# wtaylor17/ImageCFGen-Pytorch

Measured on AMD Instinct MI355X. Metric: ALI training images/sec (E+G+D step), MorphoMNIST bs=512/GPU, higher is better.
Workload: dtype f32; 1 GPU; image_scms/mnist.py ALI iteration (EG step + 2 D steps + diagnostics), MorphoMNIST 28x28x1 synthetic, bs=512/GPU, fp32 MFMA, mode=stepper+hipgraph; global_batch=512, parallelism=dp1

## Files before the change

imagecfgen-pytorch_amd/csrc/ali_common.h:

```cpp
#pragma once
#include <hip/hip_runtime.h>
#include <stdint.h>
#include <stdio.h>
#include <stdlib.h>
#include "../../include/ali_hip.h"

namespace ali {

void set_error(const char* fmt, ...);

inline int check_launch(const char* what) {
  hipError_t e = hipGetLastError();
  if (e != hipSuccess) {
    set_error("%s: %s", what, hipGetErrorString(e));
    return ALI_ERR_LAUNCH;
  }
  return ALI_OK;
}

struct Tuning {
  int bm, bn, splitk;
  long long wgrad_small;
  int wgrad_blocks, wgrad_scap;
  int no_first_wgrad;
  int no_order;
  int tile_m_scale;
  int wbm, wbn;
  int no_xcd;
  int no_s2_first;
  int no_dma16;
  int no_t1_mfma;
};
inline Tuning read_tuning() {
  {
    auto num = [](const char* name) -> long long { const char* e = getenv(name); return e ? atoll(e) : 0; };
    Tuning v;
    v.bm = (int)num("ALI_BM"); v.bn = (int)num("ALI_BN"); v.splitk = (int)num("ALI_SPLITK");
    v.wgrad_small = getenv("ALI_WGRAD_SMALL") ? num("ALI_WGRAD_SMALL") : -1;
    v.wgrad_blocks = (int)num("ALI_WGRAD_BLOCKS"); v.wgrad_scap = (int)num("ALI_WGRAD_SCAP");
    v.no_order = (int)num("ALI_NO_ORDER");
    v.no_first_wgrad = (int)num("ALI_NO_FIRST_WGRAD");
    v.tile_m_scale = (int)num("ALI_TILE_M_SCALE");
    v.wbm = (int)num("ALI_WBM"); v.wbn = (int)num("ALI_WBN");
    v.no_t1_mfma = (int)num("ALI_NO_T1_MFMA");
    v.no_xcd = (int)num("ALI_NO_XCD");
    v.no_s2_first = (int)num("ALI_NO_S2_FIRST");
    v.no_dma16 = (int)num("ALI_NO_DMA16");
    return v;
  }
}
inline Tuning& tuning_slot() {
  static Tuning t = read_tuning();
  return t;
}
inline const Tuning& tuning() { return tuning_slot(); }

using f32x4 = __attribute__((ext_vector_type(4))) float;
using f32x16 = __attribute__((ext_vector_type(16))) float;

constexpr int kMaxTaps = 28;
constexpr int kNumCU = 256;

constexpr size_t kWsReserved = ALI_WS_RESERVED;
inline void* ws_payload(void* ws) { return ws ? static_cast<char*>(ws) + kWsReserved : nullptr; }
inline size_t ws_payload_bytes(size_t bytes) { return bytes > kWsReserved ? bytes - kWsReserved : 0; }

#define ST(s) ((hipStream_t)(s))
inline bool aligned16(const void* p) { return (reinterpret_cast<uintptr_t>(p) & 15) == 0; }

constexpr uint64_t kCounterMul = 0xD1B54A32D192ED03ull;
__host__ __device__ __forceinline__ uint64_t mix64(uint64_t z) {
  z += 0x9E3779B97F4A7C15ull;
  z = (z ^ (z >> 30)) * 0xBF58476D1CE4E5B9ull;
  z = (z ^ (z >> 27)) * 0x94D049BB133111EBull;
  return z ^ (z >> 31);
}

constexpr uint64_t kLatentStream = 0x4C4154454E545A31ull;
__device__ __forceinline__ void normal_pair(uint64_t key, uint64_t pair, float& c, float& s) {
  const uint64_t r = mix64(key ^ pair);
// ... 27 lines not shown
```

imagecfgen-pytorch_amd/csrc/gconv.hip:

```cpp
#include "ali_common.h"
#include <algorithm>
#include <vector>
#include <stdarg.h>
#include <stdlib.h>
#include <string.h>
#include <type_traits>

namespace ali {

static thread_local char g_err[512] = "";
void set_error(const char* fmt, ...) {
  va_list ap;
  va_start(ap, fmt);
  vsnprintf(g_err, sizeof(g_err), fmt, ap);
  va_end(ap);
}
const char* get_error() { return g_err; }

constexpr int BK = 32;
constexpr int LDK = BK + 4;
constexpr int kMaxGrid = 5;

struct Phase {
  int Hq, Wq;
  int oh0, ow0, ostep;
  int mult;
  int nr, ns, M, tile0, pixmajor;
  signed char dh[kMaxGrid], dw[kMaxGrid];
  unsigned char wr[kMaxGrid], ws[kMaxGrid];
};

struct GDesc {
  const float* in;
  const float* w;
  float* out;
  float* ws;
  int* ctr;
  AliEpilogue ep;
  int B, Hin, Win, Cin;
  int Hout, Wout, Cout, ldo;
  int ldw, S;
  int nphase, splitk, kt_per_split;
  int ntile_m, ntile_n;
  int lin1d;
  int xcd_chunk;
  int tail_u0, tail_split;
  const int* order;
  int ldi;
  int f16;
  const _Float16* in16;
  const _Float16* w16;
  _Float16* out16;
  unsigned in_bytes, w_bytes;
  long long out_elems;
  Phase ph[4];
};

__device__ __attribute__((aligned(64))) float g_zero[16];

__device__ __forceinline__ void fast_divmod(int m, int dv, float rcp, int& q, int& r) {
  q = (int)((float)m * rcp);
  r = m - q * dv;
  if (r < 0) { --q; r += dv; }
  else if (r >= dv) { ++q; r -= dv; }
}

using f16x4 = __attribute__((ext_vector_type(4))) _Float16;
using f16x8 = __attribute__((ext_vector_type(8))) _Float16;
constexpr int LDH = 40;

template <int BM, int BN, int WAVES_M, int WAVES_N, int MODE, int F16 = 0, int NT = 256>
__device__ __forceinline__ void gconv_body(const GDesc& d, const int bx_, const int by_, const int bz_, const int u_) {
  constexpr int WM = BM / WAVES_M, WN = BN / WAVES_N;
  constexpr int TM = WM / 32, TN = WN / 32;
  constexpr int RPP = NT / 8;
  constexpr int AP = BM / RPP, BP = BN / RPP;
  constexpr bool DMA = F16 == 3;
  constexpr int LDX = DMA ? 32 : LDK;
  constexpr int NL = AP + BP;
  constexpr int NMF = 16 * TM * TN;
  static_assert(WAVES_M * WAVES_N * 64 == NT, "one wave per 64 threads");

  __shared__ __attribute__((aligned(1024))) float As[2][BM * LDX];
  __shared__ __attribute__((aligned(1024))) float Bs[2][BN * LDX];
  __shared__ int s_rowoff[BM];
  __shared__ int s_rowimg[BM];
  __shared__ int s_tap[kMaxTaps];
  __shared__ __attribute__((aligned(16))) int s_live[kMaxTaps + 8][4];
  __shared__ unsigned s_tapmask;

  const int t = threadIdx.x;
  const int lane = t & 63, wave = t >> 6;
  const int wm = wave / WAVES_N, wn = wave % WAVES_N;

  int bx = bx_, by = by_, bz = bz_, nsplit = d.splitk;
  if (d.lin1d) {
    int u = u_;
    bz = 0;
    nsplit = 1;
    if (u >= d.tail_u0) {
      const int r = u - d.tail_u0;
      u = d.tail_u0 + r / d.tail_split;
      bz = r - (r / d.tail_split) * d.tail_split;
      nsplit = d.tail_split;
    }
    if (d.xcd_chunk) {
      const int id = (u & 7) * d.xcd_chunk + (u >> 3);
      if (id >= d.ntile_m * d.ntile_n) return;
      bx = id / d.ntile_n;
      by = id - bx * d.ntile_n;
    } else if (d.order) {
      const int full = (d.ntile_m >> 3) << 3;
      int rank;
      if (u < full * d.ntile_n) {
        const int grp = u / (8 * d.ntile_n), rem = u - grp * 8 * d.ntile_n;
        rank = grp * 8 + (rem & 7);
        by = rem >> 3;
      } else {
        const int r = u - full * d.ntile_n;
        rank = full + r / d.ntile_n;
        by = r - (r / d.ntile_n) * d.ntile_n;
      }
      bx = d.order[rank];
    } else {
      by = u / d.ntile_m;
      bx = u - by * d.ntile_m;
    }
  }
  int p = 0;
#pragma unroll
  for (int i = 1; i < 4; ++i)
    if (i < d.nphase && bx >= d.ph[i].tile0) p = i;
  const Phase& P = d.ph[p];
  const int m0 = (bx - P.tile0) * BM;
  const int n0 = by * BN;
  const int Cin = d.Cin, Hin = d.Hin, Win = d.Win;
  const int ntaps = P.nr * P.ns;

  if (t < kMaxTaps) {
    int v = 0;
    if (t < ntaps) {
      const int ir = t / P.ns, is = t - ir * P.ns;
      v = (P.dh[ir] & 0xff) | ((P.dw[is] & 0xff) << 8) | (((int)P.wr[ir] * d.S + (int)P.ws[is]) << 16);
    }
    s_tap[t] = v;
  }
  if (t == 0) s_tapmask = 0u;

  const float rW = 1.0f / (float)P.Wq, rH = 1.0f / (float)P.Hq, rB = 1.0f / (float)d.B;
  auto decode = [&](int m, int& img, int& qh, int& qw) {
    if (P.pixmajor) {
      int pix;
      fast_divmod(m, d.B, rB, pix, img);
      fast_divmod(pix, P.Wq, rW, qh, qw);
    } else {
      int t2;
      fast_divmod(m, P.Wq, rW, t2, qw);
      fast_divmod(t2, P.Hq, rH, img, qh);
    }
  };
  for (int r = t; r < BM; r += NT) {
    const int m = m0 + r;
    int off = -1, img = 0;
    if (m < P.M) {
      int qh, qw;
      decode(m, img, qh, qw);
      off = ((img * d.Hout + P.oh0 + qh * P.ostep) * d.Wout + (P.ow0 + qw * P.ostep)) * d.ldo;
    }
    s_rowoff[r] = off;
    s_rowimg[r] = img;
  }

  const int c4 = t & 7;
  const int r0 = t >> 3;
  int aoff[AP], aih[AP], aiw[AP];
  unsigned amask[AP];
  unsigned blockmask = 0u;
#pragma unroll
  for (int i = 0; i < AP; ++i) {
    const int m = m0 + r0 + RPP * i;
    const bool valid = m < P.M;
    int qw, qh, img;
    decode(valid ? m : 0, img, qh, qw);
    aih[i] = qh * P.mult;
    aiw[i] = qw * P.mult;
    aoff[i] = ((img * Hin + aih[i]) * Win + aiw[i]) * d.ldi;
    unsigned wbits = 0u, mk = 0u;
    for (int is = 0; is < P.ns; ++is)
      if ((unsigned)(aiw[i] + P.dw[is]) < (unsigned)Win) wbits |= 1u << is;
    for (int ir = 0; ir < P.nr; ++ir)
      if ((unsigned)(aih[i] + P.dh[ir]) < (unsigned)Hin) mk |= wbits << (ir * P.ns);
    amask[i] = valid ? mk : 0u;
    blockmask |= amask[i];
  }
  __syncthreads();
  if (c4 == 0 && blockmask) atomicOr(&s_tapmask, blockmask);
  __syncthreads();
  const unsigned tapmask = s_tapmask;

  float bias_pre[TN];
#pragma unroll
  for (int j = 0; j < TN; ++j) {
    const int n = n0 + wn * WN + j * 32 + (lane & 31);
    bias_pre[j] = (d.ep.bias && n < d.Cout) ? d.ep.bias[n] : 0.f;
  }

  f32x16 acc[TM][TN];
#pragma unroll
  for (int i = 0; i < TM; ++i)
#pragma unroll
    for (int j = 0; j < TN; ++j)
#pragma unroll
      for (int r = 0; r < 16; ++r) acc[i][j][r] = 0.f;

  f32x4 ra[AP], rb[BP];
  f32x4 ra1[AP], rb1[BP];
  auto store_tile = [&](int buf) {
#pragma unroll
    for (int i = 0; i < AP; ++i) *reinterpret_cast<f32x4*>(&As[buf][(r0 + RPP * i) * LDK + c4 * 4]) = ra[i];
#pragma unroll
    for (int j = 0; j < BP; ++j) *reinterpret_cast<f32x4*>(&Bs[buf][(r0 + RPP * j) * LDK + c4 * 4]) = rb[j];
  };
  const int lrow = lane & 31, lh = lane >> 5;
  const float* Ab = &As[0][(wm * WM + lrow) * LDK + lh * 4];
  const float* Bb = &Bs[0][(wn * WN + lrow) * LDK + lh * 4];
  f32x4 fa[2][TM], fb[2][TN];

  if (MODE >= 2) {
    if (MODE == 3) {
      if (t < kMaxTaps + 8) {
        const bool live = t < ntaps && ((tapmask >> t) & 1u);
        const int tv = s_tap[t < kMaxTaps ? t : 0];
        const int dh = (signed char)(tv & 0xff), dw = (signed char)((tv >> 8) & 0xff), wt = (tv >> 16) & 0xff;
        s_live[t][0] = ((dh * Win + dw) * d.ldi) * 4;
        s_live[t][1] = live ? (wt * Cin) * 4 : (int)0xFFFFFF00u;
        s_live[t][2] = live ? (int)(1u << t) : 0;
        s_live[t][3] = 0;
      }
    } else if (t < ntaps && ((tapmask >> t) & 1u)) {
      const int pos = __popc(tapmask & ((1u << t) - 1u));
      const int tv = s_tap[t];
      const int dh = (signed char)(tv & 0xff), dw = (signed char)((tv >> 8) & 0xff), wt = (tv >> 16) & 0xff;
      s_live[pos][0] = ((dh * Win + dw) * d.ldi) * 4;
      s_live[pos][1] = (wt * Cin) * 4;
      s_live[pos][2] = (int)(1u << t);
      s_live[pos][3] = 0;
    }
    __syncthreads();
    const int tpt = MODE == 3 ? BK / Cin : 1;
    const int tsub = MODE == 3 ? (c4 * 4) / Cin : 0;
    const int ccol = MODE == 3 ? (c4 * 4) % Cin : c4 * 4;
    const int cpt = MODE == 3 ? 1 : Cin / BK;
    const int nlive = MODE == 3 ? (ntaps + tpt - 1) / tpt : __popc(tapmask);
    const int total = nlive * cpt;
    const int per = (total + nsplit - 1) / nsplit;
    const int qb = bz * per;
    const int qe = min(total, qb + per);

    const __amdgpu_buffer_rsrc_t rin = __builtin_amdgcn_make_buffer_rsrc((void*)d.in, 0, d.in_bytes, 0x00020000);
    const __amdgpu_buffer_rsrc_t rw = __builtin_amdgcn_make_buffer_rsrc((void*)d.w, 0, d.w_bytes, 0x00020000);
    constexpr unsigned OOB = 0xFFFFFF00u;
    unsigned aoffB[AP], woffB[BP];
#pragma unroll
    for (int i = 0; i < AP; ++i) aoffB[i] = (unsigned)(aoff[i] + ccol) * 4u;
#pragma unroll
    for (int j = 0; j < BP; ++j) {
      const int n = n0 + r0 + RPP * j;
      woffB[j] = n < d.Cout ? (unsigned)(((long long)n * d.ldw + ccol) * 4) : OOB;
    }
    struct Ctx { int doff, woff; unsigned bit; };
    auto tile_ctx = [&](int li, int ch, bool live) -> Ctx {
      const int lc = MODE == 3 ? (li < nlive ? li * tpt + tsub : 0)
                               : (li < nlive ? li : (nlive > 0 ? nlive - 1 : 0));
      const int4 ti = *reinterpret_cast<const int4*>(&s_live[lc][0]);
      if (MODE == 3 && li >= nlive) live = false;
      Ctx cx;
// ... 231 lines not shown
              for (int j = 0; j < TN; ++j)
                acc[i][j] = __builtin_amdgcn_mfma_f32_32x32x16_f16(ha[i], hb[j], acc[i][j], 0, 0, 0);
          }
          store_tile16(buf ^ 1, OTHER);
          __syncthreads();
          buf ^= 1;
          ++q;
        };
        while (q < qe) {
          iteration16(Set0{}, Set1{});
          if (q >= qe) break;
          iteration16(Set1{}, Set0{});
        }
      }
    } else if (qb < qe) {
      int q = qb;
      int li = q / cpt, ch = q - li * cpt;
      {
        const Ctx c0 = tile_ctx(li, ch, true);
#pragma unroll
        for (int i = 0; i < AP; ++i) load_a(c0, i, Set0{});
#pragma unroll
        for (int j = 0; j < BP; ++j) load_b(c0, j, Set0{});
        if (++ch == cpt) { ch = 0; ++li; }
        const Ctx c1 = tile_ctx(li, ch, q + 1 < qe);
#pragma unroll
        for (int i = 0; i < AP; ++i) load_a(c1, i, Set1{});
#pragma unroll
        for (int j = 0; j < BP; ++j) load_b(c1, j, Set1{});
      }
      store_tile(0);
      if (++ch == cpt) { ch = 0; ++li; }
      Ctx cxn = tile_ctx(li, ch, q + 2 < qe);
      __syncthreads();
      int buf = 0;
      auto iteration = [&](auto FETCH) {
        constexpr int fetch = decltype(FETCH)::value;
        const float* Ac = Ab + buf * (BM * LDK);
        const float* Bc = Bb + buf * (BN * LDK);
        float* Aw = &As[buf ^ 1][r0 * LDK + c4 * 4];
        float* Bw = &Bs[buf ^ 1][r0 * LDK + c4 * 4];
        Ctx cxn2 = cxn;
#pragma unroll
        for (int i = 0; i < TM; ++i) fa[0][i] = *reinterpret_cast<const f32x4*>(Ac + i * 32 * LDK);
#pragma unroll
        for (int j = 0; j < TN; ++j) fb[0][j] = *reinterpret_cast<const f32x4*>(Bc + j * 32 * LDK);
#pragma unroll
        for (int s = 0; s < NMF; ++s) {
          const int kg = s / (4 * TM * TN), e = (s / (TM * TN)) & 3, i = (s / TN) % TM, j = s % TN;
          acc[i][j] = __builtin_amdgcn_mfma_f32_32x32x2f32(fa[kg & 1][i][e], fb[kg & 1][j][e], acc[i][j], 0, 0, 0);
          __builtin_amdgcn_sched_barrier(0);
          {
            constexpr int Q = NMF / 4;
            if (s < Q) {
#pragma unroll
              for (int x = 0; x < NL; ++x) {
                if ((x * Q) / NL != s) continue;
                if (x < AP) load_a(cxn, x, FETCH); else load_b(cxn, x - AP, FETCH);
              }
            }
          }
          {
            const int sg = s - kg * 4 * TM * TN - 1;
            if (kg < 3 && sg >= 0 && sg < TM + TN) {
              if (sg < TM)
                fa[(kg + 1) & 1][sg] = *reinterpret_cast<const f32x4*>(Ac + sg * 32 * LDK + (kg + 1) * 8);
              else
                fb[(kg + 1) & 1][sg - TM] = *reinterpret_cast<const f32x4*>(Bc + (sg - TM) * 32 * LDK + (kg + 1) * 8);
            }
          }
          if (s == NMF / 2) {
            if (++ch == cpt) { ch = 0; ++li; }
            cxn2 = tile_ctx(li, ch, q + 3 < qe);
          }
          {
            constexpr int Q = NMF / 4;
            const int sw = s - 3 * Q;
            if (sw >= 0) {
#pragma unroll
              for (int x = 0; x < NL; ++x) {
                if ((x * Q) / NL != sw) continue;
                if (x < AP) *reinterpret_cast<f32x4*>(Aw + RPP * x * LDK) = fetch ? ra[x] : ra1[x];
                else *reinterpret_cast<f32x4*>(Bw + RPP * (x - AP) * LDK) = fetch ? rb[x - AP] : rb1[x - AP];
              }
            }
          }
          __builtin_amdgcn_sched_barrier(0);
        }
        cxn = cxn2;
        __syncthreads();
        buf ^= 1;
        ++q;
      };
      while (q < qe) {
        iteration(Set0{});
        if (q >= qe) break;
        iteration(Set1{});
      }
    }
  } else {
    const int Ktot = ntaps * Cin;
    const int nkt = (Ktot + BK - 1) / BK;
    const int kt_begin = bz * d.kt_per_split;
    const int kt_end = min(nkt, kt_begin + d.kt_per_split);
    const float* wptr[BP];
    bool bvalid[BP];
#pragma unroll
    for (int j = 0; j < BP; ++j) {
      const int n = n0 + r0 + RPP * j;
      bvalid[j] = n < d.Cout;
      wptr[j] = d.w + (long long)(bvalid[j] ? n : 0) * d.ldw;
    }
    auto tile_live = [&](int kt) -> bool {
      const int tlo = (kt * BK) / Cin;
      int thi = (kt * BK + BK - 1) / Cin;
      if (thi > ntaps - 1) thi = ntaps - 1;
      const unsigned span = (thi - tlo + 1) >= 32 ? 0xffffffffu : ((1u << (thi - tlo + 1)) - 1u);
      return ((tapmask >> tlo) & span) != 0u;
    };
    auto next_live = [&](int kt) -> int {
      while (kt < kt_end && !tile_live(kt)) ++kt;
      return kt;
    };
    auto load_tile = [&](int kt, bool live) {
      const int kflat = kt * BK + c4 * 4;
      if (MODE == 1) {
        const bool kvalid = live && kflat < Ktot;
        const int tap = kvalid ? kflat / Cin : 0;
        const int c = kflat - tap * Cin;
        const int tv = s_tap[tap];
// ... 436 lines not shown
  if (dma) S = 1;
  if (blocks > (long long)(kWsReserved / sizeof(int)) || !ws) S = 1;
  while (S > 1 && (long long)S * d.out_elems * 4 >= 0xFF000000LL) --S;
  d.splitk = S;
  d.kt_per_split = (max_nkt + S - 1) / S;
  if (d.kt_per_split < 1) d.kt_per_split = 1;
  d.ntile_m = tiles;
  d.ntile_n = ntile_n;
  d.tail_split = 1;
  d.tail_u0 = 0;
  if (S == 1 && uni && ws && blocks > kNumCU && blocks < 4 * kNumCU && blocks <= (long long)(kWsReserved / sizeof(int))
      && tuning().splitk == 0 && !dma) {
    const int R = (int)(blocks % kNumCU);
    int Sr = 1;
    while (R > 0 && Sr * 2 <= 8 && Sr * 2 * R <= kNumCU && max_nkt / (Sr * 2) >= 4) Sr *= 2;
    if (Sr > 1 && (size_t)Sr * d.out_elems * sizeof(float) <= ws_payload_bytes(ws_bytes) &&
        (long long)Sr * d.out_elems * 4 < 0xFF000000LL) {
      d.tail_split = Sr;
      d.tail_u0 = (int)(blocks - R);
    }
  }
  d.order = nullptr;
  if (d.ep.tile_order && uni && S == 1 && d.ep.tile_order_n == tiles && tuning().no_order == 0)
    d.order = reinterpret_cast<const int*>(d.ep.tile_order);
  d.lin1d = (d.tail_split > 1 || d.order) ? 1 : 0;
  if (d.tail_split == 1) d.tail_u0 = (int)blocks;
  d.xcd_chunk = 0;
  bool img_major = d.nphase >= 1;
  for (int i = 0; i < d.nphase; ++i) img_major = img_major && !d.ph[i].pixmajor;
  if (!d.lin1d && S == 1 && !job && img_major && blocks >= 8LL * kNumCU && blocks < (1LL << 30) && tuning().no_xcd == 0) {
    d.xcd_chunk = (int)((blocks + 7) / 8);
    d.lin1d = 1;
  }
  d.ctr = reinterpret_cast<int*>(ws);
  d.ws = reinterpret_cast<float*>(ws_payload(ws));
  dim3 grid(tiles, ntile_n, S), block(256);
  if (d.lin1d) grid = dim3(d.tail_u0 + (int)(blocks - d.tail_u0) * d.tail_split, 1, 1);
  if (d.xcd_chunk) grid = dim3(8 * d.xcd_chunk, 1, 1);
  if (tiles == 0 || d.out_elems == 0) return ALI_OK;
  const bool f16 = d.f16 && uni;
  const bool op16 = f16 && d.in16 && d.w16 && (d.Cin % 64) == 0;
  if (!d.f16) d.out16 = nullptr;
  if (job && uni && !f16 && ((tc.bm == 64 && tc.bn == 64) || (tc.bm == 128 && tc.bn == 32))) {
    GJobRec r;
    memset(&r, 0, sizeof(r));
    r.state = 1;
    r.variant = tc.bm == 64 ? 0 : 1;
    r.gx = (int)grid.x; r.gy = (int)grid.y; r.gz = (int)grid.z;
    r.cost = (max_nkt + S - 1) / S;
    r.d = d;
    memcpy(job, &r, sizeof(r));
    return ALI_OK;
  }
#define LAUNCH(BM_, BN_, WMM, WNN)                                                                    \
  do {                                                                                                  \
    if (op16) hipLaunchKernelGGL((gconv_kernel<BM_, BN_, WMM, WNN, 2, 2>), grid, block, 0, stream, d);  \
    else if (f16) hipLaunchKernelGGL((gconv_kernel<BM_, BN_, WMM, WNN, 2, 1>), grid, block, 0, stream, d); \
    else if (uni) hipLaunchKernelGGL((gconv_kernel<BM_, BN_, WMM, WNN, 2>), grid, block, 0, stream, d); \
    else if (pow2) hipLaunchKernelGGL((gconv_kernel<BM_, BN_, WMM, WNN, 3>), grid, block, 0, stream, d);  \
    else if (vec) hipLaunchKernelGGL((gconv_kernel<BM_, BN_, WMM, WNN, 1>), grid, block, 0, stream, d); \
    else hipLaunchKernelGGL((gconv_kernel<BM_, BN_, WMM, WNN, 0>), grid, block, 0, stream, d);          \
  } while (0)
  if (dma) {
    if (tc.bn != 256 || !op16) { set_error("gconv: no kernel for this tile"); return ALI_ERR_BAD_ARG; }
    block = dim3(512);
    hipLaunchKernelGGL((gconv_kernel512<256, 256, 2, 4, 2, 3>), grid, block, 0, stream, d);
// ... 553 lines not shown
```

imagecfgen-pytorch_amd/csrc/wgrad.hip:

```cpp
#include "ali_common.h"
#include <string.h>
#include <algorithm>
#include <vector>

namespace ali {

constexpr int WBK = 16;

struct WDesc {
  const float* x;
  const float* dy;
  float* dst;
  float* ws;
  int B, H, W, Cg, P, Q, Cd;
  int R, S, stride, pad;
  int Cg_log, Cd_log;
  long long s_dc, s_gc, s_tap;
  int Mtot;
  int npix, pix_per_split, splitk;
  long long slab;
  float* db;
  float* dbws;
  const int* pixtab;
  const _Float16* x16;
  const _Float16* dy16;
  int ldd;
};

template <int BM, int BN, int WAVES_M, int WAVES_N, bool VECA, bool VECB>
__global__ __launch_bounds__(256) void wgrad_kernel(const WDesc d) {
  constexpr int WM = BM / WAVES_M, WN = BN / WAVES_N;
  constexpr int TM = WM / 32, TN = WN / 32;
  constexpr int LDA = BM + 4, LDB = BN + 4;
  constexpr int A4 = BM / 4, B4 = BN / 4;
  constexpr int AP = (WBK * A4 + 255) / 256, BP = (WBK * B4 + 255) / 256;
  constexpr int AROWS = 256 / A4, BROWS = 256 / B4;

  __shared__ __attribute__((aligned(16))) float As[2][WBK * LDA];
  __shared__ __attribute__((aligned(16))) float Bs[2][WBK * LDB];
  __shared__ long long s_rowdst[BM];

  const int t = threadIdx.x, lane = t & 63, wave = t >> 6;
  const int wm = wave / WAVES_N, wn = wave % WAVES_N;
  const int m0 = blockIdx.x * BM, n0 = blockIdx.y * BN;
  const int pix_begin = blockIdx.z * d.pix_per_split;
  const int pix_end = min(d.npix, pix_begin + d.pix_per_split);
  const int PQ = d.P * d.Q;

  for (int r = t; r < BM; r += 256) {
    const int m = m0 + r;
    long long off = -1;
    if (m < d.Mtot) {
      const int tap = m / d.Cg, gc = m - tap * d.Cg;
      if (gc < d.Cg_log) off = gc * d.s_gc + tap * d.s_tap;
    }
    s_rowdst[r] = off;
  }

  const int a4 = t % A4, arow0 = t / A4;
// ... 124 lines not shown
    }
  }
}

constexpr int WBK2 = 32;

__device__ __forceinline__ void w_divmod(int m, int dv, float rcp, int& q, int& r) {
  q = (int)((float)m * rcp);
  r = m - q * dv;
  if (r < 0) { --q; r += dv; }
  else if (r >= dv) { ++q; r -= dv; }
}

using wf16x4 = __attribute__((ext_vector_type(4))) _Float16;
using wf16x8 = __attribute__((ext_vector_type(8))) _Float16;
typedef short ws4v __attribute__((__vector_size__(4 * sizeof(short))));

template <int BM, int BN, int WAVES_M, int WAVES_N, bool TAB, int F16 = 0>
__device__ __forceinline__ void wgrad_fast_body(const WDesc& d, const unsigned x_bytes, const unsigned dy_bytes,
                                                const int bx_, const int by_, const int bz_) {
  constexpr int WM = BM / WAVES_M, WN = BN / WAVES_N;
  constexpr int TM = WM / 32, TN = WN / 32;
  constexpr int LDA = BM + 4, LDB = BN + 4;
  constexpr int A4 = BM / 4, B4 = BN / 4;
  constexpr int AROWS = 256 / A4, BROWS = 256 / B4;
  constexpr int AP = WBK2 / AROWS, BP = WBK2 / BROWS;
  constexpr int NL = AP + BP;
  constexpr int NMF = (WBK2 / 2) * TM * TN;
  static_assert(AP >= 1 && BP >= 1, "tile");

  __shared__ __attribute__((aligned(16))) float As[2][WBK2 * LDA];
  __shared__ __attribute__((aligned(16))) float Bs[2][WBK2 * LDB];
  __shared__ long long s_rowdst[BM];

  const int t = threadIdx.x, lane = t & 63, wave = t >> 6;
  const int wm = wave / WAVES_N, wn = wave % WAVES_N;
  const int m0 = bx_ * BM, n0 = by_ * BN;
  const int pix_begin = bz_ * d.pix_per_split;
  const int pix_end = min(d.npix, pix_begin + d.pix_per_split);
  const int PQ = d.P * d.Q;
  const float rPQ = 1.0f / (float)PQ, rQ = 1.0f / (float)d.Q;

  for (int r = t; r < BM; r += 256) {
    const int m = m0 + r;
    long long off = -1;
    if (m < d.Mtot) {
      const int tap = m / d.Cg, gc = m - tap * d.Cg;
      if (gc < d.Cg_log) off = gc * d.s_gc + tap * d.s_tap;
    }
    s_rowdst[r] = off;
  }
  const int a4 = t % A4, arow0 = t / A4;
  const int mA = m0 + a4 * 4;
  const bool a_ok = mA < d.Mtot;
  const int tapA = a_ok ? mA / d.Cg : 0;
  const int gcA = mA - tapA * d.Cg;
  const int dhA = tapA / d.S - d.pad, dwA = tapA % d.S - d.pad;
  const int b4 = t % B4, brow0 = t / B4;
  const int nB = n0 + b4 * 4;
  const bool b_ok = nB < d.Cd;
  const __amdgpu_buffer_rsrc_t rx = __builtin_amdgcn_make_buffer_rsrc((void*)d.x, 0, x_bytes, 0x00020000);
  const __amdgpu_buffer_rsrc_t ry = __builtin_amdgcn_make_buffer_rsrc((void*)d.dy, 0, dy_bytes, 0x00020000);
  constexpr unsigned OOB = 0xFFFFFF00u;
  __syncthreads();

  f32x4 ra[AP], rb[BP];
  const bool do_db = d.db != nullptr && bx_ == 0;
  f32x4 dbacc = {0.f, 0.f, 0.f, 0.f};
  using i32x2 = __attribute__((ext_vector_type(2))) int;
  i32x2 te[AP];
  const __amdgpu_buffer_rsrc_t rt = __builtin_amdgcn_make_buffer_rsrc(
      (void*)d.pixtab, 0, TAB ? (unsigned)pix_end * 8u : 0u, 0x00020000);
  const int tapoffA = ((dhA * d.W + dwA) * d.Cg + gcA) * 4;
  auto load_te = [&](int pix0, int i) {
    const int pix = pix0 + arow0 + i * AROWS;
    te[i] = __builtin_bit_cast(i32x2, __builtin_amdgcn_raw_buffer_load_b64(rt, pix * 8, 0, 0));
  };
  auto load_a = [&](int pix0, int i) {
    unsigned off = OOB;
    if (TAB) {
      const int ih = (te[i].y & 0xffff) - 0x4000 + dhA, iw = (int)((unsigned)te[i].y >> 16) - 0x4000 + dwA;
      if (a_ok && (unsigned)ih < (unsigned)d.H && (unsigned)iw < (unsigned)d.W) off = (unsigned)(te[i].x + tapoffA);
    } else {
      const int pix = pix0 + arow0 + i * AROWS;
      if (a_ok && pix < pix_end) {
        int b, rem, p, q;
        w_divmod(pix, PQ, rPQ, b, rem);
        w_divmod(rem, d.Q, rQ, p, q);
        const int ih = p * d.stride + dhA, iw = q * d.stride + dwA;
        if ((unsigned)ih < (unsigned)d.H && (unsigned)iw < (unsigned)d.W)
          off = (unsigned)(((b * d.H + ih) * d.W + iw) * d.Cg + gcA) * 4u;
      }
    }
    ra[i] = __builtin_bit_cast(f32x4, __builtin_amdgcn_raw_buffer_load_b128(rx, (int)off, 0, 0));
  };
  auto load_b = [&](int pix0, int j) {
    const int pix = pix0 + brow0 + j * BROWS;
    const unsigned off = (b_ok && pix < pix_end) ? (unsigned)(pix * d.ldd + nB) * 4u : OOB;
    rb[j] = __builtin_bit_cast(f32x4, __builtin_amdgcn_raw_buffer_load_b128(ry, (int)off, 0, 0));
  };
  auto store_tile = [&](int buf) {
#pragma unroll
    for (int i = 0; i < AP; ++i) *reinterpret_cast<f32x4*>(&As[buf][(arow0 + i * AROWS) * LDA + a4 * 4]) = ra[i];
#pragma unroll
    for (int j = 0; j < BP; ++j) {
      *reinterpret_cast<f32x4*>(&Bs[buf][(brow0 + j * BROWS) * LDB + b4 * 4]) = rb[j];
      if (do_db) dbacc += rb[j];
    }
  };

  f32x16 acc[TM][TN];
#pragma unroll
  for (int i = 0; i < TM; ++i)
#pragma unroll
    for (int j = 0; j < TN; ++j)
#pragma unroll
      for (int r = 0; r < 16; ++r) acc[i][j][r] = 0.f;

  if constexpr (F16 == 2 && TAB) {
    if (pix_begin < pix_end) {
      constexpr int PA = BM + 32, PB = BN + 32;
      constexpr int A8 = BM / 8, B8 = BN / 8;
      constexpr int AROWS8 = 256 / A8, BROWS8 = 256 / B8;
      constexpr int AP8 = WBK2 / AROWS8, BP8 = WBK2 / BROWS8;
      static_assert(AP8 >= 1 && BP8 >= 1, "fp16-in-memory wgrad needs tiles of at least 64 x 64");
      _Float16* A16 = reinterpret_cast<_Float16*>(&As[0][0]);
      _Float16* B16 = reinterpret_cast<_Float16*>(&Bs[0][0]);
      const __amdgpu_buffer_rsrc_t rx16 = __builtin_amdgcn_make_buffer_rsrc((void*)d.x16, 0, x_bytes / 2, 0x00020000);
      const __amdgpu_buffer_rsrc_t ry16 = __builtin_amdgcn_make_buffer_rsrc((void*)d.dy16, 0, dy_bytes / 2, 0x00020000);
      const int a8 = t % A8, arow8 = t / A8;
      const int mA8 = m0 + a8 * 8;
// ... 172 lines not shown
#pragma unroll
          for (int i = 0; i < TM; ++i)
#pragma unroll
            for (int j = 0; j < TN; ++j)
              acc[i][j] = __builtin_amdgcn_mfma_f32_32x32x16_f16(ha[i], hb[j], acc[i][j], 0, 0, 0);
        }
        cvt_store(buf ^ 1, oa, ob);
        __syncthreads();
        buf ^= 1;
      };
      for (int pix0 = pix_begin; pix0 < pix_end;) {
        iteration16(pix0, sa0, sb0, ra1, rb1);
        pix0 += WBK2;
        if (pix0 >= pix_end) break;
        iteration16(pix0, ra1, rb1, sa0, sb0);
        pix0 += WBK2;
      }
    }
  } else if (pix_begin < pix_end) {
    if (TAB) {
#pragma unroll
      for (int i = 0; i < AP; ++i) load_te(pix_begin, i);
    }
#pragma unroll
    for (int i = 0; i < AP; ++i) load_a(pix_begin, i);
#pragma unroll
    for (int j = 0; j < BP; ++j) load_b(pix_begin, j);
    if (TAB) {
#pragma unroll
      for (int i = 0; i < AP; ++i) load_te(pix_begin + WBK2, i);
    }
    store_tile(0);
    __syncthreads();
    int buf = 0;
    const int lcol = lane & 31, lh = lane >> 5;
    float fa[2][TM], fb[2][TN];
    for (int pix0 = pix_begin; pix0 < pix_end; pix0 += WBK2) {
      const int nxt = pix0 + WBK2;
      const float* Ac = &As[buf][lh * LDA + wm * WM + lcol];
      const float* Bc = &Bs[buf][lh * LDB + wn * WN + lcol];
#pragma unroll
      for (int i = 0; i < TM; ++i) fa[0][i] = Ac[i * 32];
#pragma unroll
      for (int j = 0; j < TN; ++j) fb[0][j] = Bc[j * 32];
#pragma unroll
      for (int s = 0; s < NMF; ++s) {
        const int ks = s / (TM * TN), i = (s / TN) % TM, j = s % TN;
        acc[i][j] = __builtin_amdgcn_mfma_f32_32x32x2f32(fa[ks & 1][i], fb[ks & 1][j], acc[i][j], 0, 0, 0);
        __builtin_amdgcn_sched_barrier(0);
        {
          constexpr int Q = NMF / 4;
          if (s < Q) {
#pragma unroll
            for (int x = 0; x < NL; ++x) {
              if ((x * Q) / NL != s) continue;
              if (x < AP) load_a(nxt, x); else load_b(nxt, x - AP);
            }
          }
          if (TAB && s >= Q && s < 2 * Q) {
#pragma unroll
            for (int x = 0; x < AP; ++x)
              if ((x * Q) / AP == s - Q) load_te(nxt + WBK2, x);
          }
        }
        {
          const int sg = s - ks * TM * TN;
          if (ks + 1 < WBK2 / 2 && sg < TM + TN) {
            if (sg < TM) fa[(ks + 1) & 1][sg] = Ac[(ks + 1) * 2 * LDA + sg * 32];
            else fb[(ks + 1) & 1][sg - TM] = Bc[(ks + 1) * 2 * LDB + (sg - TM) * 32];
          }
          if (TM * TN < TM + TN && ks + 1 < WBK2 / 2 && sg == TM * TN - 1) {
#pragma unroll
            for (int x = TM * TN; x < TM + TN; ++x) {
              if (x < TM) fa[(ks + 1) & 1][x] = Ac[(ks + 1) * 2 * LDA + x * 32];
              else fb[(ks + 1) & 1][x - TM] = Bc[(ks + 1) * 2 * LDB + (x - TM) * 32];
            }
          }
        }
        {
          constexpr int Q = NMF / 4;
          const int sw = s - 3 * Q;
          if (sw >= 0) {
#pragma unroll
            for (int x = 0; x < NL; ++x) {
              if ((x * Q) / NL != sw) continue;
              if (x < AP) *reinterpret_cast<f32x4*>(&As[buf ^ 1][(arow0 + x * AROWS) * LDA + a4 * 4]) = ra[x];
              else {
                *reinterpret_cast<f32x4*>(&Bs[buf ^ 1][(brow0 + (x - AP) * BROWS) * LDB + b4 * 4]) = rb[x - AP];
                if (do_db) dbacc += rb[x - AP];
              }
            }
          }
        }
        __builtin_amdgcn_sched_barrier(0);
      }
      __syncthreads();
      buf ^= 1;
    }
  }

  const bool partial = d.splitk > 1;
  if (do_db && F16 != 2) {
    __syncthreads();
    float* red = &As[0][0];
    *reinterpret_cast<f32x4*>(&red[brow0 * BN + b4 * 4]) = dbacc;
    __syncthreads();
    if (t < BN) {
      float sum = 0.f;
      for (int r = 0; r < BROWS; ++r) sum += red[r * BN + t];
      const int n = n0 + t;
      if (n < d.Cd_log) {
        if (partial) d.dbws[(long long)bz_ * d.Cd + n] = sum;
        else d.db[n] = sum;
      }
    }
  }
  if (partial) {
#pragma unroll
    for (int j = 0; j < TN; ++j) {
      const int n = n0 + wn * WN + j * 32 + (lane & 31);
      if (n >= d.Cd) continue;
#pragma unroll
      for (int i = 0; i < TM; ++i) {
#pragma unroll
        for (int r = 0; r < 16; ++r) {
          const int m = m0 + wm * WM + i * 32 + (r & 3) + 8 * (r >> 2) + 4 * (lane >> 5);
          if (m < d.Mtot) d.ws[(long long)bz_ * d.slab + (long long)m * d.Cd + n] = acc[i][j][r];
        }
      }
// ... 392 lines not shown
      fold->T = 25; fold->reserved = 0;
      fold->ws_used = (uint64_t)kWsReserved + ((uint64_t)S * d.slab + (uint64_t)S * g->K) * sizeof(float);
      return ALI_OK;
    }
    const int T = 25, G = 1, TD = 32;
    int SGN = kRedLds / (G * T);
    if (SGN > kRedGroups) SGN = kRedGroups;
    if (SGN > S) SGN = S;
    hipLaunchKernelGGL(wgrad_reduce_tile_kernel<32>, dim3(5, (g->K + TD - 1) / TD), dim3(256), 0, stream, d.ws, S, d.Mtot, 5,
                       d.Cd, 5, Cd_log, (long long)s_dc, (long long)s_gc, (long long)s_tap, dst, d.dbws, d.db, G, T, SGN,
                       d.slab);
    return check_launch("wgrad_reduce_tile_kernel");
  }
  const int wbk = fast ? WBK2 : WBK;
  const int tiles_m = (d.Mtot + bm - 1) / bm, tiles_n = (g->K + bn - 1) / bn;
  const long long blocks = (long long)tiles_m * tiles_n;
  int S = 1;
  const int nkt = (d.npix + wbk - 1) / wbk;
  int target = 4 * kNumCU;
  if (job && fold && split_target > 0) target = split_target < kNumCU ? kNumCU : (split_target > 4 * kNumCU ? 4 * kNumCU : split_target);
  if (tuning().wgrad_blocks > 0) target = tuning().wgrad_blocks;
  if (blocks < target && nkt >= 4) {
    S = (int)((target + blocks - 1) / blocks);
    if (S > nkt / 2) S = nkt / 2;
    {
      int cap = d.npix >= (1 << 20) ? 512 : 128;
      if (tuning().wgrad_scap > 0) cap = tuning().wgrad_scap;
      if (S > cap) S = cap;
    }
    while (S > 1 && (size_t)S * (((size_t)d.Mtot + 1) * g->K + kSlabPad) * sizeof(float) > ws_bytes) --S;
    if (S < 1) S = 1;
  }
  d.splitk = S;
  int per = (nkt + S - 1) / S;
  d.pix_per_split = per * wbk;
  d.db = fast ? db : nullptr;
  d.slab = (long long)d.Mtot * g->K + kSlabPad;
  d.dbws = d.ws + (size_t)S * d.slab;
  dim3 grid(tiles_m, tiles_n, S), block(256);
  if (fast) {
    const unsigned xb = (unsigned)(x_elems * 4), yb = (unsigned)(dy_elems * 4);
    d.pixtab = (pixtab && g->H < 0x2000 && g->W < 0x2000 && g->pad < 0x2000) ? pixtab : nullptr;
    const bool f16 = mfma_f16 && d.pixtab;
    const bool mem16 = f16 && x16 && dy16 && (g->C % 8) == 0 && (g->K % 8) == 0 && bn >= 64 && d.ldd == g->K;
    d.x16 = mem16 ? reinterpret_cast<const _Float16*>(x16) : nullptr;
    d.dy16 = mem16 ? reinterpret_cast<const _Float16*>(dy16) : nullptr;
#define FLAUNCH1(BM_, BN_, WMM, WNN)                                                                              \
  do {                                                                                                            \
    if (f16) hipLaunchKernelGGL((wgrad_fast_kernel<BM_, BN_, WMM, WNN, true, 1>), grid, block, 0, stream, d, xb, yb);     \
    else if (d.pixtab) hipLaunchKernelGGL((wgrad_fast_kernel<BM_, BN_, WMM, WNN, true>), grid, block, 0, stream, d, xb, yb);   \
    else hipLaunchKernelGGL((wgrad_fast_kernel<BM_, BN_, WMM, WNN, false>), grid, block, 0, stream, d, xb, yb);   \
  } while (0)
#define FLAUNCH(BM_, BN_, WMM, WNN)                                                                               \
  do {                                                                                                            \
    if (mem16) hipLaunchKernelGGL((wgrad_fast_kernel<BM_, BN_, WMM, WNN, true, 2>), grid, block, 0, stream, d, xb, yb);   \
    else FLAUNCH1(BM_, BN_, WMM, WNN);                                                                            \
  } while (0)
    static_assert(sizeof(WJob) + 8 <= sizeof(AliWgradJob), "AliWgradJob too small");
    if (job && fold && bm == 64 && d.pixtab && !f16 && (S == 1 || g->R * g->S <= kRedRows)) {
      WJob wj;
      memset(&wj, 0, sizeof(wj));
      wj.d = d; wj.xb = xb; wj.yb = yb; wj.gx = tiles_m; wj.gy = tiles_n; wj.blk0 = S;
      job->opaque[0] = 1;
      memcpy(&job->opaque[1], &wj, sizeof(wj));
    }
    else if (bm == 64) FLAUNCH(64, 64, 2, 2);
// ... 145 lines not shown
```

Measured before the change: 80080 images/s.

## Add interior-tile fast path with simplified buffer-load addressing in conv and wgrad

Detects at block level when every row of a tile has all taps in bounds (no padding edges). For those clean tiles, the fp32 conv and wgrad main loops use a specialized path. It computes addresses as a fixed per-thread offset plus a wave-uniform scalar offset, skipping the per-iteration bounds and index recomputation. The loops are also unrolled in pairs with a compile-time buffer index. This adds shared-memory reductions, extra template instantiations and register pressure, and an env knob to disable it.

Result: faster. 82740 images/s, median of 6 (+3.3%).

```diff
diff --git a/imagecfgen-pytorch_amd/csrc/ali_common.h b/imagecfgen-pytorch_amd/csrc/ali_common.h
--- a/imagecfgen-pytorch_amd/csrc/ali_common.h
+++ b/imagecfgen-pytorch_amd/csrc/ali_common.h
@@ -29,6 +29,7 @@
   int no_xcd;
   int no_s2_first;
   int no_dma16;
+  int no_clean;
   int no_t1_mfma;
 };
 inline Tuning read_tuning() {
@@ -46,6 +47,7 @@
     v.no_xcd = (int)num("ALI_NO_XCD");
     v.no_s2_first = (int)num("ALI_NO_S2_FIRST");
     v.no_dma16 = (int)num("ALI_NO_DMA16");
+    v.no_clean = (int)num("ALI_NO_CLEAN");
     return v;
   }
 }
diff --git a/imagecfgen-pytorch_amd/csrc/gconv.hip b/imagecfgen-pytorch_amd/csrc/gconv.hip
--- a/imagecfgen-pytorch_amd/csrc/gconv.hip
+++ b/imagecfgen-pytorch_amd/csrc/gconv.hip
@@ -47,6 +47,7 @@
   int tail_u0, tail_split;
   const int* order;
   int ldi;
+  int no_clean;
   int f16;
   const _Float16* in16;
   const _Float16* w16;
@@ -88,6 +89,7 @@
   __shared__ int s_tap[kMaxTaps];
   __shared__ __attribute__((aligned(16))) int s_live[kMaxTaps + 8][4];
   __shared__ unsigned s_tapmask;
+  __shared__ int s_clean, s_dmin;
 
   const int t = threadIdx.x;
   const int lane = t & 63, wave = t >> 6;
@@ -145,7 +147,7 @@
     }
     s_tap[t] = v;
   }
-  if (t == 0) s_tapmask = 0u;
+  if (t == 0) { s_tapmask = 0u; s_clean = 1; s_dmin = 0x7fffffff; }
 
   const float rW = 1.0f / (float)P.Wq, rH = 1.0f / (float)P.Hq, rB = 1.0f / (float)d.B;
   auto decode = [&](int m, int& img, int& qh, int& qw) {
@@ -197,6 +199,12 @@
   if (c4 == 0 && blockmask) atomicOr(&s_tapmask, blockmask);
   __syncthreads();
   const unsigned tapmask = s_tapmask;
+  if (MODE == 2 && F16 == 0) {
+    bool mine = true;
+#pragma unroll
+    for (int i = 0; i < AP; ++i) mine = mine && (amask[i] & tapmask) == tapmask;
+    if (!mine) s_clean = 0;
+  }
 
   float bias_pre[TN];
 #pragma unroll
@@ -242,6 +250,7 @@
       const int tv = s_tap[t];
       const int dh = (signed char)(tv & 0xff), dw = (signed char)((tv >> 8) & 0xff), wt = (tv >> 16) & 0xff;
       s_live[pos][0] = ((dh * Win + dw) * d.ldi) * 4;
+      if (F16 == 0) atomicMin(&s_dmin, ((dh * Win + dw) * d.ldi) * 4);
       s_live[pos][1] = (wt * Cin) * 4;
       s_live[pos][2] = (int)(1u << t);
       s_live[pos][3] = 0;
@@ -539,15 +548,53 @@
       store_tile(0);
       if (++ch == cpt) { ch = 0; ++li; }
       Ctx cxn = tile_ctx(li, ch, q + 2 < qe);
+      const bool clean = F16 == 0 && MODE == 2 && d.no_clean == 0 && n0 + BN <= d.Cout &&
+                         __builtin_amdgcn_readfirstlane(s_clean) != 0;
+      struct CCtx { int sa, sb; unsigned na, nb; };
+      unsigned aoffC[AP];
+      int dmin = 0, tap_sa = 0, tap_sb = 0;
+      auto clean_tap = [&](int l) {
+        const int4 ti = *reinterpret_cast<const int4*>(&s_live[l < nlive ? l : nlive - 1][0]);
+        tap_sa = __builtin_amdgcn_readfirstlane(ti.x - dmin);
+        tap_sb = __builtin_amdgcn_readfirstlane(ti.y);
+      };
+      auto clean_ctx = [&](int c, bool live) -> CCtx {
+        CCtx cc;
+        cc.sa = tap_sa + c * (BK * 4);
+        cc.sb = tap_sb + c * (BK * 4);
+        cc.na = live ? d.in_bytes : 0u;
+        cc.nb = live ? d.w_bytes : 0u;
+        return cc;
+      };
+      CCtx ccn = {0, 0, 0u, 0u};
+      if (clean) {
+        dmin = __builtin_amdgcn_readfirstlane(s_dmin);
+#pragma unroll
+        for (int i = 0; i < AP; ++i) aoffC[i] = aoffB[i] + (unsigned)dmin;
+        clean_tap(li);
+        ccn = clean_ctx(ch, q + 2 < qe);
+      }
+      auto load_ac = [&](const CCtx& cc, int i, auto SET) {
+        const __amdgpu_buffer_rsrc_t r = __builtin_amdgcn_make_buffer_rsrc((void*)d.in, 0, cc.na, 0x00020000);
+        const f32x4 v = __builtin_bit_cast(f32x4, __builtin_amdgcn_raw_buffer_load_b128(r, (int)aoffC[i], cc.sa, 0));
+        if (decltype(SET)::value) ra1[i] = v; else ra[i] = v;
+      };
+      auto load_bc = [&](const CCtx& cc, int j, auto SET) {
+        const __amdgpu_buffer_rsrc_t r = __builtin_amdgcn_make_buffer_rsrc((void*)d.w, 0, cc.nb, 0x00020000);
+        const f32x4 v = __builtin_bit_cast(f32x4, __builtin_amdgcn_raw_buffer_load_b128(r, (int)woffB[j], cc.sb, 0));
+        if (decltype(SET)::value) rb1[j] = v; else rb[j] = v;
+      };
       __syncthreads();
-      int buf = 0;
-      auto iteration = [&](auto FETCH) {
+      auto iteration = [&](auto FETCH, auto CLEAN) {
         constexpr int fetch = decltype(FETCH)::value;
+        constexpr bool cl = decltype(CLEAN)::value;
+        constexpr int buf = fetch;
         const float* Ac = Ab + buf * (BM * LDK);
         const float* Bc = Bb + buf * (BN * LDK);
         float* Aw = &As[buf ^ 1][r0 * LDK + c4 * 4];
         float* Bw = &Bs[buf ^ 1][r0 * LDK + c4 * 4];
         Ctx cxn2 = cxn;
+        CCtx ccn2 = ccn;
 #pragma unroll
         for (int i = 0; i < TM; ++i) fa[0][i] = *reinterpret_cast<const f32x4*>(Ac + i * 32 * LDK);
 #pragma unroll
@@ -563,7 +610,11 @@
 #pragma unroll
               for (int x = 0; x < NL; ++x) {
                 if ((x * Q) / NL != s) continue;
-                if (x < AP) load_a(cxn, x, FETCH); else load_b(cxn, x - AP, FETCH);
+                if (cl) {
+                  if (x < AP) load_ac(ccn, x, FETCH); else load_bc(ccn, x - AP, FETCH);
+                } else {
+                  if (x < AP) load_a(cxn, x, FETCH); else load_b(cxn, x - AP, FETCH);
+                }
               }
             }
           }
@@ -577,8 +628,13 @@
             }
           }
           if (s == NMF / 2) {
-            if (++ch == cpt) { ch = 0; ++li; }
-            cxn2 = tile_ctx(li, ch, q + 3 < qe);
+            if (cl) {
+              if (++ch == cpt) { ch = 0; ++li; clean_tap(li); }
+              ccn2 = clean_ctx(ch, q + 3 < qe);
+            } else {
+              if (++ch == cpt) { ch = 0; ++li; }
+              cxn2 = tile_ctx(li, ch, q + 3 < qe);
+            }
           }
           {
             constexpr int Q = NMF / 4;
@@ -595,14 +651,24 @@
           __builtin_amdgcn_sched_barrier(0);
         }
         cxn = cxn2;
+        ccn = ccn2;
         __syncthreads();
-        buf ^= 1;
         ++q;
       };
-      while (q < qe) {
-        iteration(Set0{});
-        if (q >= qe) break;
-        iteration(Set1{});
+      auto run = [&](auto CLEAN) {
+        const int npair = (qe - qb) >> 1;
+#pragma unroll 1
+        for (int pr = 0; pr < npair; ++pr) {
+          iteration(Set0{}, CLEAN);
+          iteration(Set1{}, CLEAN);
+        }
+        if ((qe - qb) & 1) iteration(Set0{}, CLEAN);
+      };
+      if constexpr (MODE == 2 && F16 == 0) {
+        if (clean) run(std::true_type{});
+        else run(std::false_type{});
+      } else {
+        run(std::false_type{});
       }
     }
   } else {
@@ -1105,6 +1171,7 @@
     d.xcd_chunk = (int)((blocks + 7) / 8);
     d.lin1d = 1;
   }
+  d.no_clean = tuning().no_clean;
   d.ctr = reinterpret_cast<int*>(ws);
   d.ws = reinterpret_cast<float*>(ws_payload(ws));
   dim3 grid(tiles, ntile_n, S), block(256);
diff --git a/imagecfgen-pytorch_amd/csrc/wgrad.hip b/imagecfgen-pytorch_amd/csrc/wgrad.hip
--- a/imagecfgen-pytorch_amd/csrc/wgrad.hip
+++ b/imagecfgen-pytorch_amd/csrc/wgrad.hip
@@ -1,6 +1,7 @@
 #include "ali_common.h"
 #include <string.h>
 #include <algorithm>
+#include <type_traits>
 #include <vector>
 
 namespace ali {
@@ -25,6 +26,7 @@
   const _Float16* x16;
   const _Float16* dy16;
   int ldd;
+  int no_clean;
 };
 
 template <int BM, int BN, int WAVES_M, int WAVES_N, bool VECA, bool VECB>
@@ -215,6 +217,7 @@
   __shared__ __attribute__((aligned(16))) float As[2][WBK2 * LDA];
   __shared__ __attribute__((aligned(16))) float Bs[2][WBK2 * LDB];
   __shared__ long long s_rowdst[BM];
+  __shared__ int s_wclean;
 
   const int t = threadIdx.x, lane = t & 63, wave = t >> 6;
   const int wm = wave / WAVES_N, wn = wave % WAVES_N;
@@ -223,6 +226,8 @@
   const int pix_end = min(d.npix, pix_begin + d.pix_per_split);
   const int PQ = d.P * d.Q;
   const float rPQ = 1.0f / (float)PQ, rQ = 1.0f / (float)d.Q;
+  const int dH = __builtin_amdgcn_readfirstlane(d.H), dW = __builtin_amdgcn_readfirstlane(d.W);
+  const int ldd = __builtin_amdgcn_readfirstlane(d.ldd);
 
   for (int r = t; r < BM; r += 256) {
     const int m = m0 + r;
@@ -245,7 +250,12 @@
   const __amdgpu_buffer_rsrc_t rx = __builtin_amdgcn_make_buffer_rsrc((void*)d.x, 0, x_bytes, 0x00020000);
   const __amdgpu_buffer_rsrc_t ry = __builtin_amdgcn_make_buffer_rsrc((void*)d.dy, 0, dy_bytes, 0x00020000);
   constexpr unsigned OOB = 0xFFFFFF00u;
+  if (t == 0) s_wclean = 1;
   __syncthreads();
+  if (TAB && F16 == 0) {
+    const bool mine = a_ok && dhA >= 0 && dhA + (d.P - 1) * d.stride < d.H && dwA >= 0 && dwA + (d.Q - 1) * d.stride < d.W;
+    if (!mine) s_wclean = 0;
+  }
 
   f32x4 ra[AP], rb[BP];
   const bool do_db = d.db != nullptr && bx_ == 0;
@@ -263,7 +273,7 @@
     unsigned off = OOB;
     if (TAB) {
       const int ih = (te[i].y & 0xffff) - 0x4000 + dhA, iw = (int)((unsigned)te[i].y >> 16) - 0x4000 + dwA;
-      if (a_ok && (unsigned)ih < (unsigned)d.H && (unsigned)iw < (unsigned)d.W) off = (unsigned)(te[i].x + tapoffA);
+      if (a_ok && (unsigned)ih < (unsigned)dH && (unsigned)iw < (unsigned)dW) off = (unsigned)(te[i].x + tapoffA);
     } else {
       const int pix = pix0 + arow0 + i * AROWS;
       if (a_ok && pix < pix_end) {
@@ -271,15 +281,15 @@
         w_divmod(pix, PQ, rPQ, b, rem);
         w_divmod(rem, d.Q, rQ, p, q);
         const int ih = p * d.stride + dhA, iw = q * d.stride + dwA;
-        if ((unsigned)ih < (unsigned)d.H && (unsigned)iw < (unsigned)d.W)
-          off = (unsigned)(((b * d.H + ih) * d.W + iw) * d.Cg + gcA) * 4u;
+        if ((unsigned)ih < (unsigned)dH && (unsigned)iw < (unsigned)dW)
+          off = (unsigned)(((b * dH + ih) * dW + iw) * d.Cg + gcA) * 4u;
       }
     }
     ra[i] = __builtin_bit_cast(f32x4, __builtin_amdgcn_raw_buffer_load_b128(rx, (int)off, 0, 0));
   };
   auto load_b = [&](int pix0, int j) {
     const int pix = pix0 + brow0 + j * BROWS;
-    const unsigned off = (b_ok && pix < pix_end) ? (unsigned)(pix * d.ldd + nB) * 4u : OOB;
+    const unsigned off = (b_ok && pix < pix_end) ? (unsigned)(pix * ldd + nB) * 4u : OOB;
     rb[j] = __builtin_bit_cast(f32x4, __builtin_amdgcn_raw_buffer_load_b128(ry, (int)off, 0, 0));
   };
   auto store_tile = [&](int buf) {
@@ -518,11 +528,26 @@
     }
     store_tile(0);
     __syncthreads();
-    int buf = 0;
+    bool clean = false;
+    if constexpr (TAB && F16 == 0)
+      clean = d.no_clean == 0 && n0 + BN <= d.Cd && __builtin_amdgcn_readfirstlane(s_wclean) != 0;
+    unsigned boffC[BP];
+#pragma unroll
+    for (int j = 0; j < BP; ++j) boffC[j] = (unsigned)((brow0 + j * BROWS) * ldd + nB) * 4u;
+    auto load_ac = [&](int i) {
+      ra[i] = __builtin_bit_cast(f32x4, __builtin_amdgcn_raw_buffer_load_b128(rx, te[i].x + tapoffA, 0, 0));
+    };
+    auto load_bc = [&](int soff, int j) {
+      rb[j] = __builtin_bit_cast(f32x4, __builtin_amdgcn_raw_buffer_load_b128(ry, (int)boffC[j], soff, 0));
+    };
     const int lcol = lane & 31, lh = lane >> 5;
     float fa[2][TM], fb[2][TN];
-    for (int pix0 = pix_begin; pix0 < pix_end; pix0 += WBK2) {
+    auto iteration = [&](int pix0, auto BUF, auto CLEAN, auto DB) {
+      constexpr bool cl = decltype(CLEAN)::value;
+      const int buf = BUF;
+      const bool dbv = cl ? (bool)decltype(DB)::value : do_db;
       const int nxt = pix0 + WBK2;
+      const int soffB = cl ? __builtin_amdgcn_readfirstlane((int)((unsigned)nxt * (unsigned)ldd * 4u)) : 0;
       const float* Ac = &As[buf][lh * LDA + wm * WM + lcol];
       const float* Bc = &Bs[buf][lh * LDB + wn * WN + lcol];
 #pragma unroll
@@ -540,7 +565,11 @@
 #pragma unroll
             for (int x = 0; x < NL; ++x) {
               if ((x * Q) / NL != s) continue;
-              if (x < AP) load_a(nxt, x); else load_b(nxt, x - AP);
+              if (cl) {
+                if (x < AP) load_ac(x); else load_bc(soffB, x - AP);
+              } else {
+                if (x < AP) load_a(nxt, x); else load_b(nxt, x - AP);
+              }
             }
           }
           if (TAB && s >= Q && s < 2 * Q) {
@@ -573,7 +602,7 @@
               if (x < AP) *reinterpret_cast<f32x4*>(&As[buf ^ 1][(arow0 + x * AROWS) * LDA + a4 * 4]) = ra[x];
               else {
                 *reinterpret_cast<f32x4*>(&Bs[buf ^ 1][(brow0 + (x - AP) * BROWS) * LDB + b4 * 4]) = rb[x - AP];
-                if (do_db) dbacc += rb[x - AP];
+                if (dbv) dbacc += rb[x - AP];
               }
             }
           }
@@ -581,6 +610,31 @@
         __builtin_amdgcn_sched_barrier(0);
       }
       __syncthreads();
+    };
+    using B0 = std::integral_constant<int, 0>;
+    using B1 = std::integral_constant<int, 1>;
+    int pix0 = pix_begin;
+    if constexpr (TAB && F16 == 0) {
+      if (clean) {
+        if (do_db) {
+#pragma unroll 1
+          for (; pix0 + 3 * WBK2 <= pix_end; pix0 += 2 * WBK2) {
+            iteration(pix0, B0{}, std::true_type{}, std::true_type{});
+            iteration(pix0 + WBK2, B1{}, std::true_type{}, std::true_type{});
+          }
+        } else {
+#pragma unroll 1
+          for (; pix0 + 3 * WBK2 <= pix_end; pix0 += 2 * WBK2) {
+            iteration(pix0, B0{}, std::true_type{}, std::false_type{});
+            iteration(pix0 + WBK2, B1{}, std::true_type{}, std::false_type{});
+          }
+        }
+      }
+    }
+    int buf = 0;
+#pragma unroll 1
+    for (; pix0 < pix_end; pix0 += WBK2) {
+      iteration(pix0, buf, std::false_type{}, std::false_type{});
       buf ^= 1;
     }
   }
@@ -1039,6 +1093,7 @@
     if (S < 1) S = 1;
   }
   d.splitk = S;
+  d.no_clean = tuning().no_clean;
   int per = (nkt + S - 1) / S;
   d.pix_per_split = per * wbk;
   d.db = fast ? db : nullptr;
```
